# szbonaldo/FedMLP

Measured on AMD Instinct MI355X. Metric: images/sec/client (ICH 224x224 bs=128) at 1/2/4/8 GPUs; mAP vs ref, higher is better.
Workload: dtype f32; 1 GPU; FedMLP stage1 step, Resnet18, ICH-shaped synthetic 3x224x224, C=5, bs=128, one client per GPU, FedAvg all-reduce every 40 steps + once at end; parallelism=clients1, rccl_ranks=1, stream_mode=default: frozen teacher + weight gradients on the engine's side stream, arithmetic=fp32 operands+sums; products as 6 exact bf16 partials on the bf16 matrix pipe

## Files before the change

fedmlp_amd/_lib.py:

```python
import ctypes as C
import os

_HERE = os.path.dirname(os.path.abspath(__file__))
LIB_PATH = os.environ.get("FEDMLP_HIP_LIB") or os.path.join(_HERE, "libfedmlp_hip.so")

FM_MAX_CLASSES = 32
FM_MAX_GROUPS = 8
FM_COMM_ID_BYTES = 128


class FmConfig(C.Structure):
    _fields_ = [("model", C.c_int32), ("n_classes", C.c_int32), ("in_h", C.c_int32),
                ("in_w", C.c_int32), ("max_images", C.c_int32), ("reserved", C.c_int32 * 3),
                ("stream", C.c_void_p)]


class FmAdam(C.Structure):
    _fields_ = [("lr", C.c_float), ("beta1", C.c_float), ("beta2", C.c_float),
                ("eps", C.c_float), ("weight_decay", C.c_float)]


class FmSgd(C.Structure):
    _fields_ = [("lr", C.c_float), ("momentum", C.c_float), ("dampening", C.c_float),
                ("weight_decay", C.c_float), ("nesterov", C.c_int32)]
# ... 87 lines not shown
    "fm_comm_unique_id": (C.c_int, [C.POINTER(C.c_uint8)]),
    "fm_comm_init": (C.c_int, [_P, C.POINTER(C.c_uint8), _I32, _I32]),
    "fm_comm_destroy": (C.c_int, [_P]),
    "fm_comm_size": (C.c_int, [_P]),
    "fm_fedavg_allreduce": (C.c_int, [_P, C.c_float]),
    "fm_fedavg_tao": (C.c_int, [_P, C.POINTER(C.c_double), C.c_double, _F, C.POINTER(C.c_double)]),
    "fm_fedavg_proto": (C.c_int, [_P, _P, C.c_double, _F, _P]),
    "fm_profile_ops": (C.c_int, [_P, _I32, C.c_char_p, _I32]),
    "fm_debug_num_convs": (C.c_int, [_P]),
    "fm_debug_conv_info": (C.c_int, [_P, _I32, C.POINTER(_I32)]),
    "fm_debug_conv": (C.c_int, [_P, _I32, _I32, _P, _P, _P, _I32, _I32, _P]),
    "fm_debug_conv_fwd": (C.c_int, [_P, _I32, _P, _P, _I32, _I32, _P, _P, _P, _I32, _P, _P, _P, _P]),
    "fm_debug_block_dgrad": (C.c_int, [_P, _I32, _P, _P, _P, _I32]),
    "fm_debug_conv_planes": (C.c_int, [_P, _I32, _P, _I32, _P, _P, _P, _P, _I32, _P, _P]),
    "fm_debug_conv_arm": (C.c_int, [_P, _I32, _I32, _I32]),
    "fm_debug_pw": (C.c_int, [_P, _I32, _I32, _P, _P, _P, _I32, _I32, _P, _P, _P, _P]),
    "fm_debug_pw_fwd": (C.c_int, [_P, _I32, _P, _P, _I32, _I32, _P, _P, _P, _I32, _P, _P, _P, _P]),
    "fm_debug_proj_bwd": (C.c_int, [_P, _I32, _I32, _P, _P, _P, _P, _P, _I32, _I32, _P, _P]),
    "fm_debug_exp_bwd": (C.c_int, [_P, _I32, _P, _P, _P, _P, _P, _I32, _I32, _P, _P]),
    "fm_debug_get_grads": (C.c_int, [_P, _P]),
    "fm_debug_optim_arena": (C.c_int, [_P, _I32, C.POINTER(_P), C.POINTER(_I64)]),
    "fm_debug_entry_spans": (C.c_int, [_P, _P, _I32]),
    "fm_debug_activation": (C.c_int, [_P, _I32, _I32, _I32, _P, C.POINTER(_I32)]),
    "fm_debug_stem_masks": (C.c_int, [_P, _I32, _I32, _P, _P]),
    "fm_debug_lose_part": (C.c_int, [_I32]),
    "fm_debug_lane_delay": (C.c_int, [_P, _I32, _I64, _I32]),
    "fm_debug_lane_points": (C.c_int, [_P, C.POINTER(_I64), _I32]),
    "fm_debug_drop_wait": (C.c_int, [_P, _I32, _I32]),
    "fm_debug_ew": (C.c_int, [_P, _I32, C.POINTER(_P), C.POINTER(_I32), _F]),
    "fm_debug_eff": (C.c_int, [_P, _I32, C.POINTER(_P), C.POINTER(_I32), _F]),
# ... 58 lines not shown
```

fedmlp_amd/csrc/common.h:

```cpp
#pragma once
#include <hip/hip_runtime.h>
#include <stdint.h>

#include <stdlib.h>

typedef float f32x4 __attribute__((ext_vector_type(4)));

#ifndef FM_F32_FAST_SWISH
#define FM_F32_FAST_SWISH 1
#endif
#ifdef __HIPCC__
__device__ __forceinline__ float fm_swish_f32(float v)
{
#if FM_F32_FAST_SWISH
    return v * __builtin_amdgcn_rcpf(1.f + __expf(-v));
#else
    return v / (1.f + expf(-v));
#endif
}
#endif


#ifndef FM_MFMA_SPLIT_DEFAULT
#define FM_MFMA_SPLIT_DEFAULT 6
// ... 153 lines not shown
    int pix_per_split;
    int tilesM, tilesN, nblk_n;
    int sp;
    int nimg, Qtot, q_per_split, splits, xcd_remap;
    unsigned magW, magH;
};
struct StemRowsParams {
    const unsigned short* Xp;
    const unsigned short* Wst;
    float* Y;
    const float* scale;
    const float* shift;
    float* stats;
    int imgs, imgs_per_group, Hp, Wp, Ho, Wo, relu, sp;
    long long plane_bytes;
};
bool stem_rows_takes(int k, int stride, int cout, int hout, int wout, long long plane_bytes);
int stem_rows_stats_tiles(int imgs_per_group, int hout);
void launch_stem_rows(StemRowsParams p, hipStream_t s);
void k_stem_weight_planes(const float* w, unsigned short* dst, int Kw, hipStream_t s);
int launch_pwgrad(PwgradParams p, size_t slab_floats, hipStream_t s);
bool pwgrad_ring_takes(const PwgradParams& p);
int launch_pwgrad_ring(PwgradParams p, size_t slab_floats, hipStream_t s);
bool pwgrad_takes(int M, int Ci, int ksz, long long npix, long long xpix, int Wi, int pad);
void launch_igemm(IgemmParams p, int groups, hipStream_t s);
void launch_pconv(IgemmParams p, int groups, hipStream_t s);
bool pconv_takes(int M, int Ci, long long xp_pix, int Wi);
bool pconv_uses_ts(const IgemmParams& p);
int pconv_tile_m(int M);
int pconv_tile_n(int M);
size_t pconv_slab_floats();
bool launch_conv1x1_stream(const IgemmParams& p, int groups, hipStream_t s);
bool conv1x1_stream_takes(int Ci, int M, int Co);
int igemm_max_blocks();
// ... 14 lines not shown
```

fedmlp_amd/csrc/engine.hip:

```cpp
#include <math.h>
#include <stdio.h>
#include <string.h>

#include <algorithm>
#include <string>
#include <unordered_map>
#include <vector>

#include "../../include/fedmlp_hip.h"
#include "../../include/fedmlp_hip_debug.h"
#include "../../include/fedmlp_hip_rofl.h"
#include "../../include/fedmlp_hip_drift.h"
#include "comm.h"
#include "common.h"
#include "kernels.h"
#include "pwconv.h"

static thread_local std::string g_err;
const char* fm_last_error(void) { return g_err.c_str(); }
const char* fm_version(void) { return "fedmlp_hip 0.2 (gfx950)"; }

#define HIPCHK(x)                                                                              \
    do {                                                                                       \
        hipError_t e_ = (x);                                                                   \
// ... 931 lines not shown
        if (id < 0) { id = (int)e->op_names.size(); e->op_names.push_back(lab); e->op_ms.push_back(0); e->op_n.push_back(0); }
        a = get_ev(e); b = get_ev(e);
        on = a && b && hipEventRecord(a, st) == hipSuccess;
    }
    ~OpScope()
    {
        if (on && hipEventRecord(b, st) == hipSuccess) e->opevs.push_back({a, b, id});
    }
};
#define OP(lane, name) OpScope os_(e, lane, name)
#define LP(lane) lane_point(e, &(lane) == &e->side)

struct Prologue { const float *psc = nullptr, *psh = nullptr, *gate = nullptr; };
enum { ACT_NONE = 0, ACT_RELU = 1, ACT_SWISH = 2 };
struct Epilogue { const float *scale = nullptr, *shift = nullptr; In res; int act = ACT_NONE; };
struct FwdOps { float* stats = nullptr; Prologue pro; Epilogue epi; };

const unsigned short* scratch_planes(fm_engine* e, Lane& L, const float* x, long long npix, int C)
{
    if ((size_t)npix * C * 3 > e->xp_scratch_elems) { soft(e, hipErrorInvalidValue); return nullptr; }
    static const bool reuse = getenv("FM_DEBUG_REUSE_PLANES") && atoi(getenv("FM_DEBUG_REUSE_PLANES")) != 0;
    if (reuse && e->xp_scratch_src == x && e->xp_scratch_npix == npix) return e->xp_scratch;
    k_split_planes(x, e->xp_scratch, npix, C, L.st);
    e->xp_scratch_src = x; e->xp_scratch_npix = npix;
    return e->xp_scratch;
}
bool conv_uses_pconv(const fm_engine* e, const Conv& c, int imgs)
{
    return e->planes && c.pl_off >= 0 && pconv_takes(c.cout_p, c.cin_p, (long long)imgs * c.hin * c.win, c.win);
}

// ... 29 lines not shown
    q.npix = (long long)imgs * c.hout * c.wout; q.xpix = (long long)imgs * c.hin * c.win;
    q.M = c.cout_p; q.Nw = c.Kw;
    q.Ho = c.hout; q.Wo = c.wout; q.Hi = c.hin; q.Wi = c.win; q.Ci = c.cin_p; q.stride = c.stride; q.pad = c.pad; q.ksz = c.k;
    q.sp = e->products;
}
static void wgrad_geometry(const fm_engine* e, const Conv& c, int imgs, WgradParams& p)
{
    p.sp = e->products;
    p.M = c.cout_p; p.Nw = c.Kw;
    p.Ho = c.hout; p.Wo = c.wout; p.Hi = c.hin; p.Wi = c.win; p.Ci = c.cin_p; p.stride = c.stride;
    if (c.stem3) { p.Hi = c.Hp; p.Wi = c.Wp; }
    p.npix = imgs * c.hout * c.wout;
    if (e->model == 1 && c.cin == 3) { p.gather_k = c.k; p.gather_pad = c.pad; p.gather_kw_p = c.kw_p; }
}

enum class Arm { None, StemRows, PconvTs, PconvTap, PwConv, Igemm, IgemmStem, Pwgrad, PwgradRing, PwWgrad, WgradSkinny, WgradGeneric,
                 WgradGenericStem };

static Arm pconv_arm(const IgemmParams& geometry) { return pconv_uses_ts(geometry) ? Arm::PconvTs : Arm::PconvTap; }
static Arm fwd_arm(const fm_engine* e, const Conv& c, int imgs)
{
    if (e->stem_rows && c.stem3) return Arm::StemRows;
    if (conv_uses_pconv(e, c, imgs)) {
        IgemmParams p{};
        conv_fwd_geometry(c, p);
        return pconv_arm(p);
    }
    if (e->planes && c.cin != 3) return Arm::None;
    if (e->precision && (c.k == 1 || c.cin == 3)) return Arm::PwConv;
    return c.cin == 3 ? Arm::IgemmStem : Arm::Igemm;
}
static Arm dgrad_arm(const fm_engine* e, const Conv& c, int imgs)
{
    if (dgrad_uses_pconv(e, c, imgs)) {
        for (int k = 0; k < c.ncls; ++k) {
            IgemmParams p{};
            conv_dgrad_geometry(c, c.cls[k], p);
// ... 13 lines not shown
        return pwgrad_ring_takes(q) ? Arm::PwgradRing : Arm::Pwgrad;
    }
    if (e->planes && c.cin != 3) return Arm::None;
    if (e->precision && (c.k == 1 || c.cin == 3)) return Arm::PwWgrad;
    if (e->model == 1 && (c.k == 1 || c.cin == 3)) {
        WgradParams p{};
        wgrad_geometry(e, c, imgs, p);
        if (wgrad_skinny_takes(p)) return Arm::WgradSkinny;
    }
    return c.cin == 3 ? Arm::WgradGenericStem : Arm::WgradGeneric;
}
static int prof_family(Arm a, int M)
{
    const bool big = M >= 128;
    switch (a) {
    case Arm::StemRows: case Arm::IgemmStem: return 2;
    case Arm::PconvTs: case Arm::Igemm: return big ? 0 : 1;
    case Arm::PconvTap: return big ? 6 : 7;
    case Arm::Pwgrad: case Arm::WgradGeneric: return big ? 3 : 4;
    case Arm::WgradGenericStem: return big ? 3 : 5;
    case Arm::WgradSkinny: return 4;
    case Arm::PwgradRing: return 8;
    default: return -1;
    }
}

static int stats_tiles_for(Arm fwd, const Conv& c, int imgs_per_group, int groups, bool pro_gate)
{
    const int pix = imgs_per_group * c.hout * c.wout;
    auto tiles = [&](int bn) { return (pix + bn - 1) / bn; };
    switch (fwd) {
    case Arm::StemRows: return stem_rows_stats_tiles(imgs_per_group, c.hout);
    case Arm::PwConv: return pw_blocks(pix, groups, c.cout_p, c.cin == 3 ? c.Kw : c.cin_p, pro_gate, c.hout * c.wout);
    case Arm::PconvTs: case Arm::PconvTap: return tiles(pconv_tile_n(c.cout_p));
    default: return tiles(igemm_tile_n(c.cout_p, c.cin == 3));
    }
}

void conv_fwd(fm_engine* e, Lane& L, int ci, const Weights& W, In x, Out y, int imgs, int groups, const FwdOps& o = {})
{
    Conv& c = e->convs[ci];
    const Epilogue& ep = o.epi;
    const Prologue& pro = o.pro;
    float* const stats = o.stats;
    const Arm arm = fwd_arm(e, c, imgs);
    const int tiles_n = stats_tiles_for(arm, c, imgs / groups, groups, pro.gate != nullptr);
    if (stats) { e->stats_conv = ci; e->stats_tiles_n = tiles_n; }
    const int fam = prof_family(arm, c.cout_p);
    const double flops = 2.0 * c.macs_per_img * imgs;
    switch (arm) {
    case Arm::StemRows: {
        StemRowsParams q{};
        q.Xp = e->x3p + (size_t)e->in_img0 * c.Hp * c.Wp * 4; q.Wst = W.wst; q.Y = y.f;
        q.scale = ep.scale; q.shift = ep.shift; q.stats = stats; q.relu = ep.act;
        q.imgs = imgs; q.imgs_per_group = imgs / groups; q.Hp = c.Hp; q.Wp = c.Wp; q.Ho = c.hout; q.Wo = c.wout;
        q.sp = e->products; q.plane_bytes = e->x3p_plane_elems * 2;
        ProfScope ps(e, L, fam, flops);
        launch_stem_rows(q, L.st);
        return;
    }
    case Arm::PwConv: {
        const bool stem16 = c.cin == 3;
        PwParams q{};
        q.zeros = e->zeros;
        q.W = W.wb + c.wb_off;
        q.X = reinterpret_cast<const bf16*>(stem16 ? e->stem_col : x.f); q.Y = reinterpret_cast<bf16*>(y.f);
        if (stem16) q.X += (size_t)e->in_img0 * c.hout * c.wout * c.Kw;
        q.M = c.cout_p; q.K = stem16 ? c.Kw : c.cin_p;
        q.npix = (imgs / groups) * c.hout * c.wout; q.groups = groups;
        q.scale = ep.scale; q.shift = ep.shift; q.res = reinterpret_cast<const bf16*>(ep.res.f); q.act = ep.act;
        q.stats = stats;
// ... 249 lines not shown
}

void conv_fwd_train(fm_engine* e, Lane& L, int ci, const Weights& W, In x, int groups, int B, BnMode mode, const char* op = nullptr,
                    const Prologue& pro = {})
{
    const Out y{e->convs[ci].y};
    const FwdOps o{.stats = e->ws_stats, .pro = pro};
    if (op) {
        { OP(L, op); conv_fwd(e, L, ci, W, x, y, groups * B, groups, o); }
        { OP(L, "bn_fwd_finalize"); bn_fwd_finalize(e, L, ci, groups, B, mode); }
    } else {
        LP(L); conv_fwd(e, L, ci, W, x, y, groups * B, groups, o);
        LP(L); bn_fwd_finalize(e, L, ci, groups, B, mode);
    }
}
void conv_fwd_eval(fm_engine* e, Lane& L, int ci, const Weights& W, In x, Out y, int imgs, int act, In res = {}, const Prologue& pro = {})
{
    const int ch = e->bns[e->convs[ci].bn].ch_off;
    conv_fwd(e, L, ci, W, x, y, imgs, 1, {.pro = pro, .epi = {W.ev_scale + ch, W.ev_shift + ch, res, act}});
}

void bn_bwd_finalize(fm_engine* e, Lane& L, const Bn& b, int groups, int partials, int count, bool frozen)
{
    const BnSlots s = bn_slots(e, b);
    k_bn_bwd_finalize(e->ws_part, groups, partials, b.C, count, s.gamma, b.mean, b.istd, e->ca, e->cb, e->cc, s.dgamma, s.dbeta, L.st, frozen);
}
enum class Mask { None, Z, ZPlane, OwnOutput };
void bn_bwd(fm_engine* e, Lane& L, int bi, const float* dz, Out dy, int groups, int imgs_per_group, bool frozen, Mask mask = Mask::None,
            In z = {}, float* dyh_out = nullptr)
{
    const Conv& c = e->convs[bi];
    Bn& b = e->bns[bi];
    const int pix = imgs_per_group * c.hout * c.wout;
    const char* fy = getenv("FM_BN_MASK_FROM_Y");
// ... 115 lines not shown
            apply(blk.c2, out, idt);
        }
        cur = out;
    }
    const Conv& cl = e->convs[e->blocks.back().c2];
    LP(L); k_avgpool(cur.f, DT_F32, e->feat, imgs, cl.hout * cl.wout, 512, L.st);
    LP(L); k_fc_fwd(e->feat, S + e->off_fcw, S + e->off_fcb, e->logits, imgs, 512, e->C, L.st);
    if (mode != BnMode::Frozen) net_changed(e, e->student, Moved::Stats);
}

void forward_eval(fm_engine* e, Lane& L, Weights& W, Acts& A, int imgs, float* feat, float* logits)
{
    const float* S = W.state;
    LP(L); ensure_eval_affine(e, L, W);
    Conv& c0 = e->convs[0];
    LP(L); conv_fwd_eval(e, L, 0, W, {e->x4}, {A.stem_y}, imgs, ACT_RELU);
    LP(L);
    if (A.p0.p) k_stem_pool_planes(A.stem_y, nullptr, nullptr, A.p0.f, nullptr, A.p0.p, 1, imgs, c0.hout, c0.wout, 64, L.st);
    else k_stem_pool(A.stem_y, nullptr, nullptr, A.p0.f, nullptr, 1, imgs, c0.hout, c0.wout, 64, L.st);
    In cur = A.p0;
    for (size_t bi = 0; bi < e->blocks.size(); ++bi) {
        const Block& blk = e->blocks[bi];
        BlockActs& a = A.blk[bi];
        const bool last = bi + 1 == e->blocks.size();
        LP(L); conv_fwd_eval(e, L, blk.c1, W, cur, kept(a.z1), imgs, ACT_RELU);
        In idt = cur.f ? In{cur.f} : cur;
        if (blk.ds >= 0) {
            LP(L); conv_fwd_eval(e, L, blk.ds, W, cur, {a.ds_y}, imgs, ACT_NONE);
            idt = {a.ds_y};
        }
        const Out out = last ? Out{a.out.f} : kept(a.out);
        LP(L); conv_fwd_eval(e, L, blk.c2, W, kept(a.z1), out, imgs, ACT_RELU, idt);
        cur = out;
    }
// ... 2401 lines not shown
    ensure_packed(e);
    conv_fwd(e, e->main, conv, e->student, {.p = xp_dev}, {out_dev, outp_dev}, imgs, 1, {.epi = {scale_dev, shift_dev, {res_dev, resp_dev}, relu}});
    HIPCHK(hipStreamSynchronize(e->main.st));
    STEP_DONE(e);
    return FM_OK;
}

int fm_debug_conv_arm(fm_engine* e, int32_t op, int32_t conv, int32_t imgs)
{
    ARGCHK(e && conv >= 0 && conv < (int)e->convs.size(), "conv index");
    ARGCHK(!e->precision, "fm_debug_conv_arm: a precision-0 engine");
    ARGCHK(imgs >= 1 && imgs <= e->maxB && op >= 0 && op <= 2, "imgs / op");
    const Conv& c = e->convs[conv];
    if (op == 1 && c.cin == 3) return FM_ARM_STEM_DGRAD;
    ARGCHK(op != 1 || c.ncls > 0, "dgrad unavailable for this conv");
    switch (op == 0 ? fwd_arm(e, c, imgs) : (op == 1 ? dgrad_arm(e, c, imgs) : wgrad_arm(e, c, imgs))) {
    case Arm::StemRows: return FM_ARM_STEM_ROWS;
    case Arm::PconvTs: return FM_ARM_PCONV_TS;
    case Arm::PconvTap: return FM_ARM_PCONV_TAP;
    case Arm::Igemm: return FM_ARM_IGEMM;
    case Arm::IgemmStem: return FM_ARM_IGEMM_STEM;
    case Arm::Pwgrad: return FM_ARM_PWGRAD;
    case Arm::PwgradRing: return FM_ARM_PWGRAD_RING;
    case Arm::WgradSkinny: return FM_ARM_WGRAD_SKINNY;
    case Arm::WgradGeneric:
    case Arm::WgradGenericStem: return FM_ARM_WGRAD_GENERIC;
    default: break;
    }
    g_err = "bad argument: no kernel for this shape in planes mode";
    return FM_ERR_ARG;
}

int fm_debug_ew(fm_engine* e, int32_t op, void* const* p, const int32_t* d, const float* sc)
{
    ARGCHK(e && p && d && sc, "null argument");
    ARGCHK(e->model == 0 && !e->precision, "fm_debug_ew: a precision-0 ResNet-18 engine");
    hipStream_t s = e->main.st;
    auto F = [&](int i) { return static_cast<float*>(p[i]); };
    auto U = [&](int i) { return static_cast<unsigned short*>(p[i]); };
    auto B = [&](int i) { return static_cast<uint8_t*>(p[i]); };
    auto need = [&](std::initializer_list<int> idx) { for (int i : idx) if (!p[i]) return false; return true; };
    auto pos = [&](int n) { for (int i = 0; i < n; ++i) if (d[i] < 1) return false; return true; };
    switch (op) {
    case FM_EW_SPLIT_PLANES:
    case FM_EW_PLANES_TO_F32:
// ... 313 lines not shown
```

fedmlp_amd/csrc/planes_ew.hip:

```cpp
#include "common.h"
#include "kernels.h"
#include "split3.h"

static inline int pe_cdiv(int64_t a, int64_t b) { return (int)((a + b - 1) / b); }

#if __HIP_DEVICE_COMPILE__
__device__ __forceinline__ size_t pe_off(int c, int64_t pix, int64_t P)
{
    return (((size_t)(c >> 5) * 3) * P + pix) * 64 + ((c & 15) >> 2) * 16 + ((c >> 4) & 1) * 8;
}
__device__ __forceinline__ void pe_store_planes(unsigned short* planes, int64_t P, int c, int64_t pix, f32x4 v, bool active)
{
    f32x4 up;
#pragma unroll
    for (int k = 0; k < 4; ++k) up[k] = __shfl_down(v[k], 4);
    if (active && (c & 16) == 0) {
        sp_u32x4 H, M, L;
        split3(v, up, H, M, L);
        unsigned char* d = reinterpret_cast<unsigned char*>(planes) + (((size_t)(c >> 5) * 3) * P + pix) * 64 + ((c & 15) >> 2) * 16;
        *reinterpret_cast<sp_u32x4*>(d) = H;
        *reinterpret_cast<sp_u32x4*>(d + (size_t)P * 64) = M;
        *reinterpret_cast<sp_u32x4*>(d + (size_t)P * 128) = L;
    }
}
__device__ __forceinline__ f32x4 pe_load_planes(const unsigned short* planes, int64_t P, int c, int64_t pix)
{
    const unsigned char* s = reinterpret_cast<const unsigned char*>(planes) + pe_off(c, pix, P);
    const uint2 H = *reinterpret_cast<const uint2*>(s);
    const uint2 M = *reinterpret_cast<const uint2*>(s + (size_t)P * 64);
    const uint2 L = *reinterpret_cast<const uint2*>(s + (size_t)P * 128);
    f32x4 v;
    v[0] = (__builtin_bit_cast(float, H.x << 16) + __builtin_bit_cast(float, M.x << 16)) + __builtin_bit_cast(float, L.x << 16);
    v[1] = (__builtin_bit_cast(float, H.x & 0xffff0000u) + __builtin_bit_cast(float, M.x & 0xffff0000u)) + __builtin_bit_cast(float, L.x & 0xffff0000u);
    v[2] = (__builtin_bit_cast(float, H.y << 16) + __builtin_bit_cast(float, M.y << 16)) + __builtin_bit_cast(float, L.y << 16);
    v[3] = (__builtin_bit_cast(float, H.y & 0xffff0000u) + __builtin_bit_cast(float, M.y & 0xffff0000u)) + __builtin_bit_cast(float, L.y & 0xffff0000u);
    return v;
}
__device__ __forceinline__ f32x4 pe_mask_h(f32x4 d, const unsigned short* zh, int64_t P, int c, int64_t pix)
{
// ... 164 lines not shown
```

fedmlp_amd/csrc/stem_rows.hip:

```cpp
#include <stdlib.h>

#include <algorithm>
#include <type_traits>

#include "common.h"
#include "kernels.h"
#include "split3.h"

#if __HIP_DEVICE_COMPILE__
template <int IMM> __device__ __forceinline__ sp_u32x4 sr_lds_read128(unsigned addr)
{
    sp_u32x4 v;
    asm volatile("ds_read_b128 %0, %1 offset:%2" : "=v"(v) : "v"(addr), "n"(IMM));
    return v;
}
template <int CTRL> __device__ __forceinline__ float sr_dpp(float v)
{
    return __builtin_bit_cast(float, __builtin_amdgcn_update_dpp(0, __builtin_bit_cast(int, v), CTRL, 0xF, 0xF, false));
}
#endif

namespace {
constexpr int SR_WBYTES = 7 * 3 * 64 * 64;
constexpr int SR_PLANE = 24 * 1024;
constexpr int SR_LDS = SR_WBYTES + 3 * SR_PLANE + 4 * 64 * 2 * 4;
}

template <int SP>
__global__ __launch_bounds__(512, 2) void stem_rows_kernel(const StemRowsParams p)
{
#if __HIP_DEVICE_COMPILE__
    constexpr int FR = 2, FC = 7;
    typedef __attribute__((address_space(3))) void lds_void;
    extern __shared__ __attribute__((aligned(16))) unsigned char smem[];
    const int tid = threadIdx.x;
    const int lane = tid & 63, wave = __builtin_amdgcn_readfirstlane(tid >> 6);
    const int wm = wave >> 2, wn = wave & 3;
    const int li = lane & 15, lg = lane >> 4;
    const unsigned lds0 = (unsigned)(size_t)smem;
    const unsigned Wl = lds0, Xl = lds0 + SR_WBYTES;
    float* red = reinterpret_cast<float*>(smem + SR_WBYTES + 3 * SR_PLANE);
    constexpr unsigned OOB = 0x80000000u;
    const int Wp = p.Wp, Ho = p.Ho, Wo = p.Wo;
// ... 78 lines not shown
        for (int c = 0; c < FC; ++c) {
            float* o = p.Y + (((size_t)img * Ho + oh) * Wo + 16 * c + li) * 64;
#pragma unroll
            for (int r = 0; r < FR; ++r) {
                const int m = mbase + 16 * r;
                f32x4 v = a[r][c];
                if (p.scale) v = v * scv[r] + shv[r];
                if (p.relu == 1) {
#pragma unroll
                    for (int q = 0; q < 4; ++q) v[q] = fmaxf(v[q], 0.f);
                }
                *reinterpret_cast<f32x4*>(o + m) = v;
            }
        }
    };
    if ((int)blockIdx.x < ntiles) load_rows(blockIdx.x);
    for (int tile = blockIdx.x; tile < ntiles; tile += gridDim.x) {
        asm volatile("s_waitcnt vmcnt(0)" ::: "memory");
        __builtin_amdgcn_s_barrier();
        asm volatile("" ::: "memory");

        f32x4 acc[FR][FC];
#pragma unroll
        for (int r = 0; r < FR; ++r)
#pragma unroll
            for (int c = 0; c < FC; ++c) acc[r][c] = f32x4{0.f, 0.f, 0.f, 0.f};
        sp_u32x4 A0[FR][3], A1[FR][3], Bb[3][3];
#define SR_READA(KH, DST)                                                                        \
    {                                                                                            \
        const unsigned a_ = Af + (unsigned)((KH) * 3 * 4096);       \
        DST[0][0] = sr_lds_read128<0 * 4096>(a_);                                                 \
        DST[0][1] = sr_lds_read128<1 * 4096>(a_);                                                 \
// ... 30 lines not shown
        SR_READA(0, A0);
        SR_READB(Bf, 0, Bb[0]);
        SR_READB(Bf, 1, Bb[1]);
        SR_LGKM0();
#define SR_G(N) column(std::integral_constant<int, N>{});
#define SR_G7(N) SR_G(N) SR_G(N + 1) SR_G(N + 2) SR_G(N + 3) SR_G(N + 4) SR_G(N + 5) SR_G(N + 6)
        SR_G7(0) SR_G7(7) SR_G7(14) SR_G7(21) SR_G7(28) SR_G7(35) SR_G7(42)
#undef SR_G7
#undef SR_G
#undef SR_MFMA
#undef SR_READB
#undef SR_READA
        asm volatile("s_waitcnt lgkmcnt(0)" ::: "memory");
        __builtin_amdgcn_s_barrier();
        asm volatile("" ::: "memory");
        if (tile + (int)gridDim.x < ntiles) load_rows(tile + gridDim.x);

        epilogue(acc, tile);
    }
#undef SR_LGKM0
#endif
}

__global__ __launch_bounds__(256) void stem_weight_planes_kernel(const float* __restrict__ w, unsigned short* __restrict__ dst, int Kw)
{
#if __HIP_DEVICE_COMPILE__
    const int idx = blockIdx.x * 256 + threadIdx.x;
    if (idx >= 7 * 64 * 4) return;
    const int g = idx & 3, m = (idx >> 2) & 63, kh = idx >> 8;
    float v[8];
#pragma unroll
    for (int e = 0; e < 8; ++e) {
        const int kw = 2 * g + (e >> 2), c = e & 3;
// ... 19 lines not shown
int stem_rows_stats_tiles(int imgs_per_group, int hout) { return imgs_per_group * (hout / 4); }

void launch_stem_rows(StemRowsParams p, hipStream_t s)
{
    static bool attr_done = false;
    if (!attr_done) {
        set_max_dyn_lds(reinterpret_cast<const void*>(&stem_rows_kernel<6>), SR_LDS, "stem_rows_kernel<6>");
        set_max_dyn_lds(reinterpret_cast<const void*>(&stem_rows_kernel<9>), SR_LDS, "stem_rows_kernel<9>");
        attr_done = true;
    }
    const int ntiles = p.imgs * (p.Ho / 4);
    const int nblk = std::min(256, ntiles);
    if (p.sp == 9) hipLaunchKernelGGL((stem_rows_kernel<9>), dim3(nblk), dim3(512), SR_LDS, s, p);
    else hipLaunchKernelGGL((stem_rows_kernel<6>), dim3(nblk), dim3(512), SR_LDS, s, p);
}
```

fedmlp_amd/engine.py:

```python
import ctypes as C

import numpy as np
import torch

from . import _lib, spec

MODEL_IDS = {"Resnet18": 0, "Efficient_b0": 1}
PRECISION_IDS = {"fp32": 0, "bf16": 1}
PRODUCT_FORMS = {None: 0, 6: 3, 0: 1, 9: 2}


def _ptr(t):
    if t is None:
        return None
    assert t.is_cuda and t.is_contiguous() and t.dtype in (torch.float32, torch.int32, torch.bfloat16), \
        (t.device, t.dtype, t.is_contiguous())
    return C.c_void_p(t.data_ptr())


def _cargs(args):
    return [_ptr(a) if torch.is_tensor(a) else a for a in args]


class RoflHeads:
# ... 753 lines not shown
    def debug_conv_fwd(self, conv, x, out, imgs, groups=1, scale=None, shift=None, res=None, act=0, psc=None, psh=None,
                       gate=None, stats=None):
        self._enqueue()
        _lib.check(self.lib.fm_debug_conv_fwd(self.h, conv, _ptr(x), _ptr(out), imgs, groups, _ptr(scale), _ptr(shift),
                                              _ptr(res), int(act), _ptr(psc), _ptr(psh), _ptr(gate), _ptr(stats)))

    def debug_conv_planes(self, conv, xp, imgs, scale, shift, res=None, resp=None, relu=0, out=None, outp=None):
        def words(t):
            assert t is None or (t.is_cuda and t.is_contiguous() and t.dtype == torch.int16), "planes are int16 device tensors"
            return None if t is None else C.c_void_p(t.data_ptr())
        self._enqueue()
        _lib.check(self.lib.fm_debug_conv_planes(self.h, conv, words(xp), imgs, _ptr(scale), _ptr(shift), _ptr(res), words(resp),
                                                 int(relu), _ptr(out), words(outp)))

    CONV_ARMS = ("igemm", "igemm_stem", "stem_rows", "pconv_ts", "pconv_tap", "pwgrad", "pwgrad_ring", "wgrad_generic",
                 "wgrad_skinny", "stem_dgrad")

    def debug_conv_arm(self, op, conv, imgs):
        rc = self.lib.fm_debug_conv_arm(self.h, op, conv, imgs)
        if rc < 0:
            _lib.check(rc)
        return self.CONV_ARMS[rc]

    def debug_block_dgrad(self, block, dy1, dyd, dx, imgs):
        self._enqueue()
        _lib.check(self.lib.fm_debug_block_dgrad(self.h, block, _ptr(dy1), _ptr(dyd), _ptr(dx), imgs))

    EW_OPS = ("split_planes", "planes_to_f32", "bn_finalize", "bn_finalize_frozen", "bn_eval_affine", "bn_apply",
              "bn_apply_planes", "stem_pool", "stem_pool_planes", "stem_pool_bwd", "stem_pool_bn_reduce", "stem_pool_bn_apply",
              "bn_bwd_reduce", "bn_bwd_finalize", "bn_bwd_apply", "bn_bwd_apply_planes")

    def debug_ew(self, op, ptrs, dims, scalars=()):
        assert len(ptrs) <= 12 and len(dims) <= 5 and len(scalars) <= 2, (len(ptrs), len(dims), len(scalars))
        for t in ptrs:
            assert t is None or (t.is_cuda and t.is_contiguous()), op
        p = (C.c_void_p * 12)(*[None if t is None else t.data_ptr() for t in ptrs])
        d = (C.c_int32 * 5)(*[int(v) for v in dims])
# ... 85 lines not shown
```

include/fedmlp_hip_debug.h:

```cpp
#ifndef FEDMLP_HIP_DEBUG_H
#define FEDMLP_HIP_DEBUG_H

#include "fedmlp_hip.h"

#ifdef __cplusplus
extern "C" {
#endif

int fm_debug_conv_info(fm_engine* e, int32_t conv, int32_t* info16);
int fm_debug_num_convs(fm_engine* e);
int fm_debug_conv(fm_engine* e, int32_t op, int32_t conv, const float* x_dev, const float* dy_dev,
                  float* out_dev, int32_t imgs, int32_t groups, float* stats_dev);

int fm_debug_conv_fwd(fm_engine* e, int32_t conv, const float* x_dev, float* out_dev, int32_t imgs, int32_t groups,
                      const float* scale_dev, const float* shift_dev, const float* res_dev, int32_t act, const float* psc_dev,
                      const float* psh_dev, const float* gate_dev, float* stats_dev);

int fm_debug_conv_planes(fm_engine* e, int32_t conv, const uint16_t* xp_dev, int32_t imgs, const float* scale_dev,
                         const float* shift_dev, const float* res_dev, const uint16_t* resp_dev, int32_t relu, float* out_dev,
                         uint16_t* outp_dev);

enum { FM_ARM_IGEMM = 0, FM_ARM_IGEMM_STEM, FM_ARM_STEM_ROWS, FM_ARM_PCONV_TS, FM_ARM_PCONV_TAP, FM_ARM_PWGRAD, FM_ARM_PWGRAD_RING,
       FM_ARM_WGRAD_GENERIC, FM_ARM_WGRAD_SKINNY, FM_ARM_STEM_DGRAD };
int fm_debug_conv_arm(fm_engine* e, int32_t op, int32_t conv, int32_t imgs);

int fm_debug_block_dgrad(fm_engine* e, int32_t block, const float* dy1_dev, const float* dyd_dev, float* dx_dev, int32_t imgs);

int fm_debug_pw(fm_engine* e, int32_t op, int32_t conv, const void* x_dev, const void* dy_dev, void* out_dev,
                int32_t imgs, int32_t groups, const float* psc_dev, const float* psh_dev, const float* gate_dev,
                float* stats_dev);

int fm_debug_pw_fwd(fm_engine* e, int32_t conv, const void* x_dev, void* out_dev, int32_t imgs, int32_t groups,
                    const float* scale_dev, const float* shift_dev, const void* res_dev, int32_t act, const float* psc_dev,
                    const float* psh_dev, const float* gate_dev, float* stats_dev);

int fm_debug_proj_bwd(fm_engine* e, int32_t conv, int32_t phase, const void* dyp_dev, const void* yd_dev, const float* bn_dev,
                      const float* gate_dev, const float* ds_dev, int32_t imgs, int32_t groups, void* out_dev,
                      float* pool5_dev);

// ... 50 lines not shown
```

Before: 6161 images/sec.

## Fuse stem BN-ReLU and 3x3 maxpool into stem_rows kernel for eval teacher

Adds a pooled variant of the stem_rows conv kernel. Each block walks all row tiles of one image in order, applies the BN affine and ReLU, and computes the 3x3/2 maxpool in LDS, carrying a halo row between tiles. The pooled result goes straight to fp32 and/or bf16 planes, so the frozen-teacher forward never writes the full stem activation and skips the separate pool kernel. The grid is limited to one block per image up to the CU count and is used only when the load balances, which gives up some tile-level parallelism and adds LDS traffic and barriers to the epilogue.

```diff
diff --git a/fedmlp_amd/_lib.py b/fedmlp_amd/_lib.py
--- a/fedmlp_amd/_lib.py
+++ b/fedmlp_amd/_lib.py
@@ -125,6 +125,7 @@
     "fm_debug_block_dgrad": (C.c_int, [_P, _I32, _P, _P, _P, _I32]),
     "fm_debug_conv_planes": (C.c_int, [_P, _I32, _P, _I32, _P, _P, _P, _P, _I32, _P, _P]),
     "fm_debug_conv_arm": (C.c_int, [_P, _I32, _I32, _I32]),
+    "fm_debug_stem_pool_eval": (C.c_int, [_P, _P, _I32, _P, _P, _P, _P, _I32, _I32]),
     "fm_debug_pw": (C.c_int, [_P, _I32, _I32, _P, _P, _P, _I32, _I32, _P, _P, _P, _P]),
     "fm_debug_pw_fwd": (C.c_int, [_P, _I32, _P, _P, _I32, _I32, _P, _P, _P, _I32, _P, _P, _P, _P]),
     "fm_debug_proj_bwd": (C.c_int, [_P, _I32, _I32, _P, _P, _P, _P, _P, _I32, _I32, _P, _P]),
diff --git a/fedmlp_amd/csrc/common.h b/fedmlp_amd/csrc/common.h
--- a/fedmlp_amd/csrc/common.h
+++ b/fedmlp_amd/csrc/common.h
@@ -191,10 +191,16 @@
     float* stats;
     int imgs, imgs_per_group, Hp, Wp, Ho, Wo, relu, sp;
     long long plane_bytes;
+    float* pool;
+    unsigned short* poolp;
+    long long pool_pix;
 };
 bool stem_rows_takes(int k, int stride, int cout, int hout, int wout, long long plane_bytes);
 int stem_rows_stats_tiles(int imgs_per_group, int hout);
 void launch_stem_rows(StemRowsParams p, hipStream_t s);
+int stem_rows_pooled_blocks(int imgs);
+bool stem_rows_pooled_pays(int imgs);
+void launch_stem_rows_pooled(StemRowsParams p, int blocks, hipStream_t s);
 void k_stem_weight_planes(const float* w, unsigned short* dst, int Kw, hipStream_t s);
 int launch_pwgrad(PwgradParams p, size_t slab_floats, hipStream_t s);
 bool pwgrad_ring_takes(const PwgradParams& p);
diff --git a/fedmlp_amd/csrc/engine.hip b/fedmlp_amd/csrc/engine.hip
--- a/fedmlp_amd/csrc/engine.hip
+++ b/fedmlp_amd/csrc/engine.hip
@@ -969,7 +969,7 @@
 struct Prologue { const float *psc = nullptr, *psh = nullptr, *gate = nullptr; };
 enum { ACT_NONE = 0, ACT_RELU = 1, ACT_SWISH = 2 };
 struct Epilogue { const float *scale = nullptr, *shift = nullptr; In res; int act = ACT_NONE; };
-struct FwdOps { float* stats = nullptr; Prologue pro; Epilogue epi; };
+struct FwdOps { float* stats = nullptr; Prologue pro; Epilogue epi; Out pool; };
 
 const unsigned short* scratch_planes(fm_engine* e, Lane& L, const float* x, long long npix, int C)
 {
@@ -1029,13 +1029,17 @@
     if (e->model == 1 && c.cin == 3) { p.gather_k = c.k; p.gather_pad = c.pad; p.gather_kw_p = c.kw_p; }
 }
 
-enum class Arm { None, StemRows, PconvTs, PconvTap, PwConv, Igemm, IgemmStem, Pwgrad, PwgradRing, PwWgrad, WgradSkinny, WgradGeneric,
+enum class Arm { None, StemRows, StemRowsPooled, PconvTs, PconvTap, PwConv, Igemm, IgemmStem, Pwgrad, PwgradRing, PwWgrad, WgradSkinny, WgradGeneric,
                  WgradGenericStem };
 
 static Arm pconv_arm(const IgemmParams& geometry) { return pconv_uses_ts(geometry) ? Arm::PconvTs : Arm::PconvTap; }
-static Arm fwd_arm(const fm_engine* e, const Conv& c, int imgs)
-{
-    if (e->stem_rows && c.stem3) return Arm::StemRows;
+static Arm fwd_arm(const fm_engine* e, const Conv& c, int imgs, bool pooled_out = false)
+{
+    if (e->stem_rows && c.stem3) {
+        const char* fu = getenv("FM_STEM_POOL_FUSED");
+        const bool fused = pooled_out && (fu ? atoi(fu) != 0 : true) && stem_rows_pooled_pays(imgs);
+        return fused ? Arm::StemRowsPooled : Arm::StemRows;
+    }
     if (conv_uses_pconv(e, c, imgs)) {
         IgemmParams p{};
         conv_fwd_geometry(c, p);
@@ -1079,7 +1083,7 @@
 {
     const bool big = M >= 128;
     switch (a) {
-    case Arm::StemRows: case Arm::IgemmStem: return 2;
+    case Arm::StemRows: case Arm::StemRowsPooled: case Arm::IgemmStem: return 2;
     case Arm::PconvTs: case Arm::Igemm: return big ? 0 : 1;
     case Arm::PconvTap: return big ? 6 : 7;
     case Arm::Pwgrad: case Arm::WgradGeneric: return big ? 3 : 4;
@@ -1096,6 +1100,7 @@
     auto tiles = [&](int bn) { return (pix + bn - 1) / bn; };
     switch (fwd) {
     case Arm::StemRows: return stem_rows_stats_tiles(imgs_per_group, c.hout);
+    case Arm::StemRowsPooled: return 0;
     case Arm::PwConv: return pw_blocks(pix, groups, c.cout_p, c.cin == 3 ? c.Kw : c.cin_p, pro_gate, c.hout * c.wout);
     case Arm::PconvTs: case Arm::PconvTap: return tiles(pconv_tile_n(c.cout_p));
     default: return tiles(igemm_tile_n(c.cout_p, c.cin == 3));
@@ -1108,18 +1113,26 @@
     const Epilogue& ep = o.epi;
     const Prologue& pro = o.pro;
     float* const stats = o.stats;
-    const Arm arm = fwd_arm(e, c, imgs);
+    const Arm arm = fwd_arm(e, c, imgs, o.pool.f || o.pool.p);
     const int tiles_n = stats_tiles_for(arm, c, imgs / groups, groups, pro.gate != nullptr);
     if (stats) { e->stats_conv = ci; e->stats_tiles_n = tiles_n; }
     const int fam = prof_family(arm, c.cout_p);
     const double flops = 2.0 * c.macs_per_img * imgs;
     switch (arm) {
-    case Arm::StemRows: {
+    case Arm::StemRows: case Arm::StemRowsPooled: {
         StemRowsParams q{};
         q.Xp = e->x3p + (size_t)e->in_img0 * c.Hp * c.Wp * 4; q.Wst = W.wst; q.Y = y.f;
         q.scale = ep.scale; q.shift = ep.shift; q.stats = stats; q.relu = ep.act;
         q.imgs = imgs; q.imgs_per_group = imgs / groups; q.Hp = c.Hp; q.Wp = c.Wp; q.Ho = c.hout; q.Wo = c.wout;
         q.sp = e->products; q.plane_bytes = e->x3p_plane_elems * 2;
+        if (arm == Arm::StemRowsPooled) {
+            if (!ep.scale || !ep.shift || ep.act != ACT_RELU || stats || groups != 1) { soft(e, hipErrorInvalidValue); return; }
+            q.Y = nullptr;
+            q.pool = o.pool.f; q.poolp = o.pool.p; q.pool_pix = (long long)imgs * (c.hout / 2) * (c.wout / 2);
+            ProfScope ps(e, L, fam, flops);
+            launch_stem_rows_pooled(q, 0, L.st);
+            return;
+        }
         ProfScope ps(e, L, fam, flops);
         launch_stem_rows(q, L.st);
         return;
@@ -1399,10 +1412,11 @@
         LP(L); bn_fwd_finalize(e, L, ci, groups, B, mode);
     }
 }
-void conv_fwd_eval(fm_engine* e, Lane& L, int ci, const Weights& W, In x, Out y, int imgs, int act, In res = {}, const Prologue& pro = {})
+void conv_fwd_eval(fm_engine* e, Lane& L, int ci, const Weights& W, In x, Out y, int imgs, int act, In res = {}, const Prologue& pro = {},
+                   Out pool = {})
 {
     const int ch = e->bns[e->convs[ci].bn].ch_off;
-    conv_fwd(e, L, ci, W, x, y, imgs, 1, {.pro = pro, .epi = {W.ev_scale + ch, W.ev_shift + ch, res, act}});
+    conv_fwd(e, L, ci, W, x, y, imgs, 1, {.pro = pro, .epi = {W.ev_scale + ch, W.ev_shift + ch, res, act}, .pool = pool});
 }
 
 void bn_bwd_finalize(fm_engine* e, Lane& L, const Bn& b, int groups, int partials, int count, bool frozen)
@@ -1548,10 +1562,12 @@
     const float* S = W.state;
     LP(L); ensure_eval_affine(e, L, W);
     Conv& c0 = e->convs[0];
-    LP(L); conv_fwd_eval(e, L, 0, W, {e->x4}, {A.stem_y}, imgs, ACT_RELU);
-    LP(L);
-    if (A.p0.p) k_stem_pool_planes(A.stem_y, nullptr, nullptr, A.p0.f, nullptr, A.p0.p, 1, imgs, c0.hout, c0.wout, 64, L.st);
-    else k_stem_pool(A.stem_y, nullptr, nullptr, A.p0.f, nullptr, 1, imgs, c0.hout, c0.wout, 64, L.st);
+    LP(L); conv_fwd_eval(e, L, 0, W, {e->x4}, {A.stem_y}, imgs, ACT_RELU, {}, {}, A.p0);
+    if (fwd_arm(e, c0, imgs, true) != Arm::StemRowsPooled) {
+        LP(L);
+        if (A.p0.p) k_stem_pool_planes(A.stem_y, nullptr, nullptr, A.p0.f, nullptr, A.p0.p, 1, imgs, c0.hout, c0.wout, 64, L.st);
+        else k_stem_pool(A.stem_y, nullptr, nullptr, A.p0.f, nullptr, 1, imgs, c0.hout, c0.wout, 64, L.st);
+    }
     In cur = A.p0;
     for (size_t bi = 0; bi < e->blocks.size(); ++bi) {
         const Block& blk = e->blocks[bi];
@@ -3983,8 +3999,9 @@
     const Conv& c = e->convs[conv];
     if (op == 1 && c.cin == 3) return FM_ARM_STEM_DGRAD;
     ARGCHK(op != 1 || c.ncls > 0, "dgrad unavailable for this conv");
-    switch (op == 0 ? fwd_arm(e, c, imgs) : (op == 1 ? dgrad_arm(e, c, imgs) : wgrad_arm(e, c, imgs))) {
+    switch (op == 0 ? fwd_arm(e, c, imgs, true) : (op == 1 ? dgrad_arm(e, c, imgs) : wgrad_arm(e, c, imgs))) {
     case Arm::StemRows: return FM_ARM_STEM_ROWS;
+    case Arm::StemRowsPooled: return FM_ARM_STEM_ROWS_POOLED;
     case Arm::PconvTs: return FM_ARM_PCONV_TS;
     case Arm::PconvTap: return FM_ARM_PCONV_TAP;
     case Arm::Igemm: return FM_ARM_IGEMM;
@@ -3998,6 +4015,38 @@
     }
     g_err = "bad argument: no kernel for this shape in planes mode";
     return FM_ERR_ARG;
+}
+
+int fm_debug_stem_pool_eval(fm_engine* e, const float* x_dev, int32_t imgs, const float* scale_dev, const float* shift_dev,
+                            float* pooled_f32_out, uint16_t* pooled_planes_out, int32_t form, int32_t blocks)
+{
+    ARGCHK(e && x_dev && scale_dev && shift_dev, "null argument");
+    ARGCHK(e->model == 0 && !e->precision && e->stem_rows, "fm_debug_stem_pool_eval: a planes-mode precision-0 ResNet-18 handle whose stem stem_rows takes");
+    ARGCHK(imgs >= 1 && imgs <= e->maxB, "imgs");
+    ARGCHK(pooled_f32_out || pooled_planes_out, "an output: fp32, planes or both");
+    ARGCHK(form == 0 || form == 1, "form");
+    ARGCHK(blocks >= 0 && blocks <= imgs && (form == 1 || blocks == 0), "blocks: 0, or the pooled form's grid of at most imgs blocks");
+    Conv& c = e->convs[0];
+    Lane& L = e->main;
+    k_frame_nhwc3(x_dev, e->x3, imgs, c.hin, c.win, c.Hp, c.Wp, 3, 3, 1, L.st, e->x3p, e->x3p_plane_elems);
+    ensure_packed(e);
+    if (form == 0) {
+        conv_fwd(e, L, 0, e->student, {x_dev}, {e->acts.stem_y}, imgs, 1, {.epi = {scale_dev, shift_dev, {}, ACT_RELU}});
+        if (pooled_planes_out)
+            k_stem_pool_planes(e->acts.stem_y, nullptr, nullptr, pooled_f32_out, nullptr, pooled_planes_out, 1, imgs, c.hout, c.wout, 64, L.st);
+        else k_stem_pool(e->acts.stem_y, nullptr, nullptr, pooled_f32_out, nullptr, 1, imgs, c.hout, c.wout, 64, L.st);
+    } else {
+        StemRowsParams q{};
+        q.Xp = e->x3p; q.Wst = e->student.wst;
+        q.scale = scale_dev; q.shift = shift_dev; q.relu = ACT_RELU;
+        q.imgs = imgs; q.imgs_per_group = imgs; q.Hp = c.Hp; q.Wp = c.Wp; q.Ho = c.hout; q.Wo = c.wout;
+        q.sp = e->products; q.plane_bytes = e->x3p_plane_elems * 2;
+        q.pool = pooled_f32_out; q.poolp = pooled_planes_out; q.pool_pix = (long long)imgs * (c.hout / 2) * (c.wout / 2);
+        launch_stem_rows_pooled(q, blocks, L.st);
+    }
+    HIPCHK(hipStreamSynchronize(L.st));
+    STEP_DONE(e);
+    return FM_OK;
 }
 
 int fm_debug_ew(fm_engine* e, int32_t op, void* const* p, const int32_t* d, const float* sc)
diff --git a/fedmlp_amd/csrc/planes_ew.hip b/fedmlp_amd/csrc/planes_ew.hip
--- a/fedmlp_amd/csrc/planes_ew.hip
+++ b/fedmlp_amd/csrc/planes_ew.hip
@@ -1,28 +1,11 @@
 #include "common.h"
 #include "kernels.h"
+#include "planes_io.h"
 #include "split3.h"
 
 static inline int pe_cdiv(int64_t a, int64_t b) { return (int)((a + b - 1) / b); }
 
 #if __HIP_DEVICE_COMPILE__
-__device__ __forceinline__ size_t pe_off(int c, int64_t pix, int64_t P)
-{
-    return (((size_t)(c >> 5) * 3) * P + pix) * 64 + ((c & 15) >> 2) * 16 + ((c >> 4) & 1) * 8;
-}
-__device__ __forceinline__ void pe_store_planes(unsigned short* planes, int64_t P, int c, int64_t pix, f32x4 v, bool active)
-{
-    f32x4 up;
-#pragma unroll
-    for (int k = 0; k < 4; ++k) up[k] = __shfl_down(v[k], 4);
-    if (active && (c & 16) == 0) {
-        sp_u32x4 H, M, L;
-        split3(v, up, H, M, L);
-        unsigned char* d = reinterpret_cast<unsigned char*>(planes) + (((size_t)(c >> 5) * 3) * P + pix) * 64 + ((c & 15) >> 2) * 16;
-        *reinterpret_cast<sp_u32x4*>(d) = H;
-        *reinterpret_cast<sp_u32x4*>(d + (size_t)P * 64) = M;
-        *reinterpret_cast<sp_u32x4*>(d + (size_t)P * 128) = L;
-    }
-}
 __device__ __forceinline__ f32x4 pe_load_planes(const unsigned short* planes, int64_t P, int c, int64_t pix)
 {
     const unsigned char* s = reinterpret_cast<const unsigned char*>(planes) + pe_off(c, pix, P);
diff --git a/fedmlp_amd/csrc/planes_io.h b/fedmlp_amd/csrc/planes_io.h
--- /dev/null
+++ b/fedmlp_amd/csrc/planes_io.h
@@ -0,0 +1,24 @@
+#pragma once
+#include "common.h"
+#include "split3.h"
+
+#if __HIP_DEVICE_COMPILE__
+__device__ __forceinline__ size_t pe_off(int c, int64_t pix, int64_t P)
+{
+    return (((size_t)(c >> 5) * 3) * P + pix) * 64 + ((c & 15) >> 2) * 16 + ((c >> 4) & 1) * 8;
+}
+__device__ __forceinline__ void pe_store_planes(unsigned short* planes, int64_t P, int c, int64_t pix, f32x4 v, bool active)
+{
+    f32x4 up;
+#pragma unroll
+    for (int k = 0; k < 4; ++k) up[k] = __shfl_down(v[k], 4);
+    if (active && (c & 16) == 0) {
+        sp_u32x4 H, M, L;
+        split3(v, up, H, M, L);
+        unsigned char* d = reinterpret_cast<unsigned char*>(planes) + (((size_t)(c >> 5) * 3) * P + pix) * 64 + ((c & 15) >> 2) * 16;
+        *reinterpret_cast<sp_u32x4*>(d) = H;
+        *reinterpret_cast<sp_u32x4*>(d + (size_t)P * 64) = M;
+        *reinterpret_cast<sp_u32x4*>(d + (size_t)P * 128) = L;
+    }
+}
+#endif
diff --git a/fedmlp_amd/csrc/stem_rows.hip b/fedmlp_amd/csrc/stem_rows.hip
--- a/fedmlp_amd/csrc/stem_rows.hip
+++ b/fedmlp_amd/csrc/stem_rows.hip
@@ -5,6 +5,7 @@
 
 #include "common.h"
 #include "kernels.h"
+#include "planes_io.h"
 #include "split3.h"
 
 #if __HIP_DEVICE_COMPILE__
@@ -24,9 +25,96 @@
 constexpr int SR_WBYTES = 7 * 3 * 64 * 64;
 constexpr int SR_PLANE = 24 * 1024;
 constexpr int SR_LDS = SR_WBYTES + 3 * SR_PLANE + 4 * 64 * 2 * 4;
-}
-
-template <int SP>
+constexpr int SR_PROW = 56 * 64 * 4;
+static_assert(5 * SR_PROW <= 3 * SR_PLANE, "the halo and four pooled half-rows live in the input rows' area");
+}
+
+#if __HIP_DEVICE_COMPILE__
+template <int FR, int FC>
+__device__ __forceinline__ void sr_pool_epilogue(const StemRowsParams& p, unsigned char* const rows, const f32x4 (&a)[FR][FC],
+                                                 f32x4 (&halo)[FC], int img, int t4, int tid, int wm, int wn, int li, int lg)
+{
+    const int mbase = 32 * wm + 4 * lg;
+    f32x4 scv[FR], shv[FR];
+#pragma unroll
+    for (int r = 0; r < FR; ++r) {
+        scv[r] = *reinterpret_cast<const f32x4*>(p.scale + mbase + 16 * r);
+        shv[r] = *reinterpret_cast<const f32x4*>(p.shift + mbase + 16 * r);
+    }
+    f32x4 h[FC], rot_prev[FR] = {};
+#pragma unroll
+    for (int c = 0; c < FC; ++c) {
+        f32x4 hm[FR];
+#pragma unroll
+        for (int r = 0; r < FR; ++r) {
+            f32x4 v = a[r][c] * scv[r] + shv[r];
+#pragma unroll
+            for (int q = 0; q < 4; ++q) v[q] = fmaxf(v[q], 0.f);
+            f32x4 rot;
+#pragma unroll
+            for (int q = 0; q < 4; ++q) {
+                rot[q] = sr_dpp<0x121>(v[q]);
+                const float nxt = sr_dpp<0x101>(v[q]);
+                const float lft = li ? rot[q] : (c ? rot_prev[r][q] : -INFINITY);
+                float b = -INFINITY;
+                if (lft > b) b = lft;
+                if (v[q] > b) b = v[q];
+                if (nxt > b) b = nxt;
+                hm[r][q] = b;
+            }
+            rot_prev[r] = rot;
+        }
+#pragma unroll
+        for (int q = 0; q < 4; ++q) {
+            const float up = sr_dpp<0x121>(hm[1][q]);
+            h[c][q] = (li & 1) ? up : hm[0][q];
+        }
+    }
+    const int chunk = (8 * wm + 4 * (li & 1) + lg) ^ ((li >> 1) << 1);
+    unsigned char* const wr = rows + (li >> 1) * 256 + chunk * 16;
+    if (wn == 3) {
+        if (t4 > 0) {
+#pragma unroll
+            for (int c = 0; c < FC; ++c) *reinterpret_cast<f32x4*>(wr + c * 2048) = halo[c];
+        }
+#pragma unroll
+        for (int c = 0; c < FC; ++c) halo[c] = h[c];
+    }
+#pragma unroll
+    for (int c = 0; c < FC; ++c) *reinterpret_cast<f32x4*>(wr + (wn + 1) * SR_PROW + c * 2048) = h[c];
+    asm volatile("s_waitcnt lgkmcnt(0)" ::: "memory");
+    __builtin_amdgcn_s_barrier();
+    asm volatile("" ::: "memory");
+#pragma unroll
+    for (int it = 0; it < 4; ++it) {
+        const int i = it * 512 + tid;
+        const bool active = i < 2 * 56 * 16;
+        const int ii = active ? i : 0;
+        const int cq = ii & 15, px = ii >> 4, prow = px >= 56 ? 1 : 0, pw = px - 56 * prow;
+        const unsigned char* rd = rows + 2 * prow * SR_PROW + pw * 256 + ((cq ^ ((pw & 7) << 1)) << 4);
+        f32x4 win[3];
+#pragma unroll
+        for (int kh = 0; kh < 3; ++kh) win[kh] = *reinterpret_cast<const f32x4*>(rd + kh * SR_PROW);
+        const bool top = prow == 0 && t4 == 0;
+        f32x4 best = {-INFINITY, -INFINITY, -INFINITY, -INFINITY};
+#pragma unroll
+        for (int kh = 0; kh < 3; ++kh)
+#pragma unroll
+            for (int k = 0; k < 4; ++k) {
+                const float u = (kh == 0 && top) ? -INFINITY : win[kh][k];
+                if (u > best[k]) best[k] = u;
+            }
+        const int64_t pix = ((int64_t)img * (p.Ho >> 1) + 2 * t4 + prow) * 56 + pw;
+        if (p.pool && active) *reinterpret_cast<f32x4*>(p.pool + pix * 64 + 4 * cq) = best;
+        if (p.poolp) pe_store_planes(p.poolp, p.pool_pix, 4 * cq, pix, best, active);
+    }
+    asm volatile("s_waitcnt lgkmcnt(0)" ::: "memory");
+    __builtin_amdgcn_s_barrier();
+    asm volatile("" ::: "memory");
+}
+#endif
+
+template <int SP, bool POOL = false>
 __global__ __launch_bounds__(512, 2) void stem_rows_kernel(const StemRowsParams p)
 {
 #if __HIP_DEVICE_COMPILE__
@@ -135,8 +223,20 @@
             }
         }
     };
-    if ((int)blockIdx.x < ntiles) load_rows(blockIdx.x);
-    for (int tile = blockIdx.x; tile < ntiles; tile += gridDim.x) {
+    f32x4 halo[POOL ? FC : 1];
+    if constexpr (POOL) {
+#pragma unroll
+        for (int c = 0; c < FC; ++c) halo[c] = f32x4{0.f, 0.f, 0.f, 0.f};
+    }
+    auto next_tile = [&](int tile) {
+        if constexpr (POOL) {
+            const int t4 = tile % tiles_per_img;
+            return t4 + 1 < tiles_per_img ? tile + 1 : tile + 1 + ((int)gridDim.x - 1) * tiles_per_img;
+        } else return tile + (int)gridDim.x;
+    };
+    const int tile0 = POOL ? (int)blockIdx.x * tiles_per_img : (int)blockIdx.x;
+    if (tile0 < ntiles) load_rows(tile0);
+    for (int tile = tile0; tile < ntiles; tile = next_tile(tile)) {
         asm volatile("s_waitcnt vmcnt(0)" ::: "memory");
         __builtin_amdgcn_s_barrier();
         asm volatile("" ::: "memory");
@@ -197,9 +297,15 @@
         asm volatile("s_waitcnt lgkmcnt(0)" ::: "memory");
         __builtin_amdgcn_s_barrier();
         asm volatile("" ::: "memory");
-        if (tile + (int)gridDim.x < ntiles) load_rows(tile + gridDim.x);
-
-        epilogue(acc, tile);
+        if constexpr (POOL) {
+            const int img = tile / tiles_per_img;
+            sr_pool_epilogue<FR, FC>(p, smem + SR_WBYTES, acc, halo, img, tile - img * tiles_per_img, tid, wm, wn, li, lg);
+            if (next_tile(tile) < ntiles) load_rows(next_tile(tile));
+        } else {
+            if (next_tile(tile) < ntiles) load_rows(next_tile(tile));
+
+            epilogue(acc, tile);
+        }
     }
 #undef SR_LGKM0
 #endif
@@ -249,3 +355,33 @@
     if (p.sp == 9) hipLaunchKernelGGL((stem_rows_kernel<9>), dim3(nblk), dim3(512), SR_LDS, s, p);
     else hipLaunchKernelGGL((stem_rows_kernel<6>), dim3(nblk), dim3(512), SR_LDS, s, p);
 }
+
+static int sr_cus()
+{
+    static int cus = 0;
+    if (!cus) {
+        int dev = 0, n = 0;
+        if (hipGetDevice(&dev) != hipSuccess || hipDeviceGetAttribute(&n, hipDeviceAttributeMultiprocessorCount, dev) != hipSuccess || n < 1)
+            return 256;
+        cus = n;
+    }
+    return cus;
+}
+int stem_rows_pooled_blocks(int imgs) { return std::min(sr_cus(), imgs); }
+bool stem_rows_pooled_pays(int imgs)
+{
+    const long long blocks = stem_rows_pooled_blocks(imgs);
+    return imgs >= sr_cus() && 8 * ((imgs + blocks - 1) / blocks) * blocks <= 9LL * imgs;
+}
+void launch_stem_rows_pooled(StemRowsParams p, int blocks, hipStream_t s)
+{
+    static bool attr_done = false;
+    if (!attr_done) {
+        set_max_dyn_lds(reinterpret_cast<const void*>(&stem_rows_kernel<6, true>), SR_LDS, "stem_rows_kernel<6, true>");
+        set_max_dyn_lds(reinterpret_cast<const void*>(&stem_rows_kernel<9, true>), SR_LDS, "stem_rows_kernel<9, true>");
+        attr_done = true;
+    }
+    const int nblk = std::min(blocks > 0 ? blocks : stem_rows_pooled_blocks(p.imgs), p.imgs);
+    if (p.sp == 9) hipLaunchKernelGGL((stem_rows_kernel<9, true>), dim3(nblk), dim3(512), SR_LDS, s, p);
+    else hipLaunchKernelGGL((stem_rows_kernel<6, true>), dim3(nblk), dim3(512), SR_LDS, s, p);
+}
diff --git a/fedmlp_amd/engine.py b/fedmlp_amd/engine.py
--- a/fedmlp_amd/engine.py
+++ b/fedmlp_amd/engine.py
@@ -791,13 +791,20 @@
                                                  int(relu), _ptr(out), words(outp)))
 
     CONV_ARMS = ("igemm", "igemm_stem", "stem_rows", "pconv_ts", "pconv_tap", "pwgrad", "pwgrad_ring", "wgrad_generic",
-                 "wgrad_skinny", "stem_dgrad")
+                 "wgrad_skinny", "stem_dgrad", "stem_rows_pooled")
 
     def debug_conv_arm(self, op, conv, imgs):
         rc = self.lib.fm_debug_conv_arm(self.h, op, conv, imgs)
         if rc < 0:
             _lib.check(rc)
         return self.CONV_ARMS[rc]
+
+    def debug_stem_pool_eval(self, x, imgs, scale, shift, pooled=None, pooledp=None, form=0, blocks=0):
+        assert pooledp is None or (pooledp.is_cuda and pooledp.is_contiguous() and pooledp.dtype == torch.int16)
+        self._enqueue()
+        _lib.check(self.lib.fm_debug_stem_pool_eval(self.h, _ptr(x), int(imgs), _ptr(scale), _ptr(shift), _ptr(pooled),
+                                                    None if pooledp is None else C.c_void_p(pooledp.data_ptr()), int(form),
+                                                    int(blocks)))
 
     def debug_block_dgrad(self, block, dy1, dyd, dx, imgs):
         self._enqueue()
diff --git a/include/fedmlp_hip_debug.h b/include/fedmlp_hip_debug.h
--- a/include/fedmlp_hip_debug.h
+++ b/include/fedmlp_hip_debug.h
@@ -21,8 +21,11 @@
                          uint16_t* outp_dev);
 
 enum { FM_ARM_IGEMM = 0, FM_ARM_IGEMM_STEM, FM_ARM_STEM_ROWS, FM_ARM_PCONV_TS, FM_ARM_PCONV_TAP, FM_ARM_PWGRAD, FM_ARM_PWGRAD_RING,
-       FM_ARM_WGRAD_GENERIC, FM_ARM_WGRAD_SKINNY, FM_ARM_STEM_DGRAD };
+       FM_ARM_WGRAD_GENERIC, FM_ARM_WGRAD_SKINNY, FM_ARM_STEM_DGRAD, FM_ARM_STEM_ROWS_POOLED };
 int fm_debug_conv_arm(fm_engine* e, int32_t op, int32_t conv, int32_t imgs);
+
+int fm_debug_stem_pool_eval(fm_engine* e, const float* x_dev, int32_t imgs, const float* scale_dev, const float* shift_dev,
+                            float* pooled_f32_out, uint16_t* pooled_planes_out, int32_t form, int32_t blocks);
 
 int fm_debug_block_dgrad(fm_engine* e, int32_t block, const float* dy1_dev, const float* dyd_dev, float* dx_dev, int32_t imgs);
 
```

Result: no change. 6163 images/sec, median of 2 (+0.0%).
